# caojiezhang/CiaoSR

Measured on AMD Instinct MI355X. Metric: HR Mpix/s (RDN-CiaoSR x4, LocalImplicitSR forward_test), higher is better.
Workload: dtype f32; 1 GPU; C3: RDN-CiaoSR (c64b16) x4, LR 1356x2040 -> 5424x8160 (DIV2K-shaped 2K LR), tiled inference: 117 tiles of 192x192 (overlap 32), random-init weights, fp32; scale=4, tiles=117, parallelism=tile-shard x1

## Files before the change

ciaosr_amd/_lib.py:

```python
import ctypes as C
import os

_HERE = os.path.dirname(os.path.abspath(__file__))
LIB_PATH = os.environ.get('CIAOSR_HIP_LIB') or os.path.join(_HERE, 'csrc', 'libciaosr_hip.so')
MAX_LAYERS = 8

ACT_NONE, ACT_RELU, ACT_PRELU, ACT_GELU, ACT_SIN, ACT_COS = 0, 1, 2, 3, 4, 5


class CiaoSRHipError(RuntimeError):
    pass


class MlpT(C.Structure):
    _fields_ = [('n_layers', C.c_int), ('act', C.c_int), ('in_dim', C.c_int), ('width', C.c_int * MAX_LAYERS),
                ('weight', C.c_void_p * MAX_LAYERS), ('ld', C.c_int * MAX_LAYERS),
                ('bias', C.c_void_p * MAX_LAYERS), ('frag', C.c_void_p * MAX_LAYERS),
                ('frag16', C.c_void_p * MAX_LAYERS), ('frag16_lo', C.c_void_p * MAX_LAYERS)]


class HeadWeightsT(C.Structure):
    _fields_ = [('channels', C.c_int), ('nonlocal_channels', C.c_int), ('nonlocal_max_scale', C.c_int), ('local_size', C.c_int),
                ('no_unfold', C.c_int),
                ('softmax_scale', C.c_float), ('q', MlpT), ('k', MlpT), ('v', MlpT), ('k_out_wino', C.c_void_p), ('k_out_wino4', C.c_void_p),
                ('chain16', C.c_void_p), ('chain16_pairs', C.c_void_p)]


class HeadSceneT(C.Structure):
    _fields_ = [(n, C.c_int) for n in ('magic', 'H', 'W', 'C', 'Cn', 'D', 'Dv', 'J', 'q_plan', 'precision', 'route',
                                       'off_u', 'off_tk', 'off_tv', 'off_g', 'total')]


class CsAttnWeightsT(C.Structure):
    _fields_ = [('channels', C.c_int), ('scale', C.c_int),
                ('w_match1', C.c_void_p), ('b_match1', C.c_void_p), ('slope_match1', C.c_float),
                ('w_match2', C.c_void_p), ('b_match2', C.c_void_p), ('slope_match2', C.c_float),
                ('w_assembly', C.c_void_p), ('b_assembly', C.c_void_p), ('slope_assembly', C.c_float),
                ('w_down', C.c_void_p), ('b_down', C.c_void_p), ('w_down_masked', C.c_void_p),
                ('escape_nan', C.c_float), ('softmax_scale', C.c_float)]


class OptionsT(C.Structure):
    _fields_ = [('head_route', C.c_int), ('csa_composed_min', C.c_int), ('dense_min_tiles', C.c_int),
                ('scatter_small_max', C.c_int), ('kv_rows', C.c_int), ('decode_rows', C.c_int), ('bf16_single', C.c_int),
                ('dense_direct', C.c_int), ('csa_scores_gemm', C.c_int), ('csa_attn_tile128', C.c_int), ('query_grid_w', C.c_int), ('f16_pairs', C.c_int),
                ('csa_attn_v16', C.c_int), ('swin_h16', C.c_int), ('csa_block_mb', C.c_int)]


HEAD_STAGED, HEAD_NO_LOGIT_TABLE, HEAD_TABLE_GEMM, HEAD_WIDE_WG, HEAD_TABLE_WINO2, HEAD_NO_CHAIN, HEAD_NO_DECODE_CHAIN = 1, 2, 4, 8, 16, 32, 64


class ConvT(C.Structure):
    _fields_ = [('weight', C.c_void_p), ('bias', C.c_void_p), ('cin', C.c_int), ('cout', C.c_int), ('ksize', C.c_int),
                ('frag16', C.c_void_p), ('frag16_lo', C.c_void_p), ('frag', C.c_void_p), ('frag_wino', C.c_void_p),
                ('frag_wino4', C.c_void_p)]


class RdnWeightsT(C.Structure):
    _fields_ = [('mid_channels', C.c_int), ('growth', C.c_int), ('num_blocks', C.c_int), ('num_layers', C.c_int),
                ('sfe1', ConvT), ('sfe2', ConvT), ('gff0', ConvT), ('gff1', ConvT),
                ('dense', C.POINTER(ConvT)), ('lff', C.POINTER(ConvT)),
                ('scatter_weight', C.POINTER(C.c_void_p)), ('scatter_bias', C.c_void_p),
                ('scatter_frag', C.POINTER(C.c_void_p))]


class SwinBlockT(C.Structure):
    _fields_ = [(n, C.c_void_p) for n in ('ln1_w', 'ln1_b', 'qkv_w', 'qkv_b', 'bias', 'proj_w', 'proj_b', 'ln2_w', 'ln2_b',
                                           'fc1_w', 'fc1_b', 'fc2_w', 'fc2_b')] + [('shift', C.c_int), ('mask', C.c_void_p)] + \
               [(n, C.c_void_p) for n in ('qkv_w16', 'proj_w16', 'fc1_w16', 'fc2_w16')]


class SwinirWeightsT(C.Structure):
    _fields_ = [('embed_dim', C.c_int), ('num_heads', C.c_int), ('window_size', C.c_int), ('hidden', C.c_int),
                ('num_groups', C.c_int), ('depth', C.c_int), ('conv_first', ConvT), ('conv_after_body', ConvT),
                ('pe_norm_w', C.c_void_p), ('pe_norm_b', C.c_void_p), ('norm_w', C.c_void_p), ('norm_b', C.c_void_p),
                ('blocks', C.POINTER(SwinBlockT)), ('group_conv', C.POINTER(ConvT))]


class EdsrWeightsT(C.Structure):
    _fields_ = [('mid_channels', C.c_int), ('num_blocks', C.c_int), ('res_scale', C.c_float),
                ('conv_first', ConvT), ('conv_after_body', ConvT),
                ('conv1', C.POINTER(ConvT)), ('conv2', C.POINTER(ConvT))]
# ... 133 lines not shown
```

ciaosr_amd/csrc/common.h:

```cpp
#pragma once
#include <hip/hip_runtime.h>
#include <atomic>
#include <cstdint>
#include <cstdio>
#include <mutex>

#include "../../include/ciaosr_hip.h"

namespace ciaosr {

constexpr int kWave = 64;

static inline int ceil_div(long a, long b) { return (int)((a + b - 1) / b); }

static inline bool aligned16(const void* p) { return (reinterpret_cast<uintptr_t>(p) & 15u) == 0; }

struct ProfScope {
    int slot;
    hipStream_t stream;
    hipEvent_t ev0, ev1;
    ProfScope(const char* name, hipStream_t s);
    ~ProfScope();
};

constexpr int kMaxDevices = 32;
struct LdsAttrOnce {
    std::atomic<unsigned> granted[kMaxDevices];
    std::mutex raise;
};
template <typename K>
static inline bool allow_big_lds(LdsAttrOnce& once, K kernel, size_t bytes) {
    if (bytes <= 64 * 1024) return true;
    int dev = 0;
    if (hipGetDevice(&dev) != hipSuccess || dev < 0 || dev >= kMaxDevices) return false;
    if (once.granted[dev].load(std::memory_order_acquire) >= bytes) return true;
    std::lock_guard<std::mutex> lock(once.raise);
    if (once.granted[dev].load(std::memory_order_relaxed) >= bytes) return true;
    if (hipFuncSetAttribute(reinterpret_cast<const void*>(kernel), hipFuncAttributeMaxDynamicSharedMemorySize, (int)bytes) !=
        hipSuccess)
        return false;
    once.granted[dev].store((unsigned)bytes, std::memory_order_release);
    return true;
}

__device__ __forceinline__ void wave_lds_sync() {
    __builtin_amdgcn_fence(__ATOMIC_RELEASE, "wavefront");
    __builtin_amdgcn_wave_barrier();
    __builtin_amdgcn_fence(__ATOMIC_ACQUIRE, "wavefront");
}

int launch_status(const char* what);

static inline bool options_ok(const ciaosr_options_t* o) {
    if (!o) return true;
    return o->query_grid_w >= 0 && (o->csa_attn_tile128 == 0 || o->csa_attn_tile128 == 1) && (o->head_route & ~127) == 0 && (o->kv_rows == 0 || o->kv_rows == 32 || o->kv_rows == 64) &&
           (o->decode_rows == 0 || o->decode_rows == 32 || o->decode_rows == 64) && (o->bf16_single == 0 || o->bf16_single == 1) &&
           (o->dense_direct >= 0 && o->dense_direct <= 2) && (o->csa_scores_gemm == 0 || o->csa_scores_gemm == 1) &&
           o->f16_pairs >= 0 && o->f16_pairs <= 3 && (o->csa_attn_v16 == 0 || o->csa_attn_v16 == 1) && o->csa_block_mb >= 0 &&
           (o->swin_h16 == 0 || o->swin_h16 == 1);
}

}

#define CIAOSR_BIG_LDS(kernel, bytes)                                                              \
    do {                                                                                           \
        static ::ciaosr::LdsAttrOnce once_;                                                        \
        if (!::ciaosr::allow_big_lds(once_, kernel, bytes)) return CIAOSR_ERR_LAUNCH;              \
    } while (0)

#define CIAOSR_CHECK_ARG(cond)                                                         \
    do {                                                                               \
        if (!(cond)) {                                                                 \
            std::fprintf(stderr, "[ciaosr_hip] bad argument: %s (%s:%d)\n", #cond,     \
                         __FILE__, __LINE__);                                          \
            return CIAOSR_ERR_BAD_ARG;                                                 \
        }                                                                              \
    } while (0)
```

ciaosr_amd/csrc/head.hip:

```cpp
#include "ops.h"

namespace ciaosr {

struct HeadPlan {
    int H, W, C, Cn, D, Dv, J, HW;
    long Q;
    int wk0, wv0;
    int wmax;
    int qc;
    int qcf;
    size_t csa_bytes;
    size_t R() const { return (size_t)qc * J; }
};

constexpr int kLdG = 260;
constexpr int kQkChunk = 65536;

static int n_samples(int local_size) { return local_size == 1 ? 1 : (local_size == 2 ? 4 : 9); }

static HeadPlan head_plan(int H, int W, const ciaosr_head_weights_t* w, int Q, const ciaosr_options_t* opt) {
    HeadPlan p;
    p.H = H; p.W = W; p.C = w->channels; p.Cn = w->nonlocal_channels; p.Q = Q;
    p.D = (w->no_unfold ? 1 : 9) * p.C; p.Dv = p.D + p.Cn; p.J = n_samples(w->local_size); p.HW = H * W;
    p.wk0 = w->k.width[0];
// ... 75 lines not shown
    return {{round_up(a[0].off, 256), round_up(a[1].off, 256), round_up(a[2].off, 256)}};
}

static int mlp_act(const ciaosr_mlp_t& m) { return m.act == CIAOSR_ACT_SIN || m.act == CIAOSR_ACT_COS ? m.act : CIAOSR_ACT_RELU; }

static bool mlp_ok(const ciaosr_mlp_t& m) {
    if (m.n_layers < 1 || m.n_layers > CIAOSR_MAX_LAYERS) return false;
    for (int i = 0; i < m.n_layers; ++i)
        if (!m.weight[i] || !m.bias[i] || (m.ld[i] & 3) != 0 || m.width[i] <= 0) return false;
    return true;
}

static bool chain_fused_ok(const ciaosr_mlp_t& m, bool is_q, bool h16) {
    if (m.n_layers < 2 || mlp_act(m) != CIAOSR_ACT_RELU) return false;
    for (int i = 0; i + 1 < m.n_layers; ++i)
        if (m.width[i] != 256) return false;
    for (int i = is_q ? 0 : 1; i < m.n_layers - (is_q ? 1 : 0); ++i)
        if (!(h16 ? m.frag16[i] : (const void*)m.frag[i])) return false;
    return true;
}

enum HeadTables { kTablesH16, kTablesSmall, kTablesGemm };
enum HeadLogit { kLogitNone, kLogitGemm32, kLogitGemm16, kLogitWino2, kLogitWino4 };
enum HeadKernel { kHeadFused32, kHeadFused16, kHeadWide, kHeadChain };
struct HeadRoute {
    int refusal;
    bool fused;
    bool h16, lo;
    HeadTables tables;
    HeadLogit logit;
    HeadKernel kernel;
    int wide_mode;
    bool chain, decode_chain;
    HeadKernel kv(const HeadPlan& p, int nq) const { return chain && (size_t)nq * p.Dv * 2 < 0xFFFFFF00ull ? kHeadChain : kernel; }
    HeadKernel decode(const HeadPlan& p, int nq) const { return decode_chain && kv(p, nq) == kHeadChain ? kHeadChain : kernel; }
};

static HeadRoute head_route(const HeadPlan& p, Prec prec, const Mode& m, const ciaosr_options_t* opt, const ciaosr_head_weights_t* w) {
    const int bits = opt ? opt->head_route : 0;
    HeadRoute r = {CIAOSR_OK, false, prec != kF32, m.lo, kTablesGemm, kLogitNone, kHeadFused32, m.x3 ? 2 : (m.lo ? 1 : 0), false, false};
    r.fused = !(bits & CIAOSR_HEAD_STAGED) && w->local_size == 2 && chain_fused_ok(w->k, false, r.h16) && chain_fused_ok(w->v, false, r.h16) &&
              chain_fused_ok(w->q, true, r.h16) && (p.Dv & 7) == 0;
    if (r.h16 && !r.fused) r.refusal = CIAOSR_ERR_UNSUPPORTED;
    if (m.x3 && r.refusal == CIAOSR_OK) {
        bool all = true;
        for (int i = 1; i < w->k.n_layers; ++i) all = all && w->k.frag16_lo[i];
        for (int i = 1; i < w->v.n_layers; ++i) all = all && w->v.frag16_lo[i];
        for (int i = 0; i + 1 < w->q.n_layers; ++i) all = all && w->q.frag16_lo[i];
        if (!all) r.refusal = CIAOSR_ERR_BAD_ARG;
    }
    if (m.hoist16 && (p.D & 7) == 0 && (p.Dv & 7) == 0 && u16_fits(p)) r.tables = kTablesH16;
    else if (gemm_small_ok(p.HW, p.wk0, p.D, p.Dv, w->k.ld[0]) && gemm_small_ok(p.HW, p.wv0, p.Dv, p.Dv, w->v.ld[0]) && p.HW <= 4096)
        r.tables = kTablesSmall;
    const int last = w->k.n_layers - 1;
    if (r.fused && !(bits & CIAOSR_HEAD_NO_LOGIT_TABLE) && w->k.width[last] == p.D && w->k.width[last - 1] == 256 && p.Q * p.J > (long)p.HW * 9 &&
        (size_t)p.HW * 9 * kLdG * sizeof(float) < 0xFFFFFF00ull) {
        r.logit = m.table16 && (p.D & 7) == 0 ? kLogitGemm16 : kLogitGemm32;
        if (!m.table16 && w->k_out_wino && !(bits & CIAOSR_HEAD_TABLE_GEMM) && p.C == 64 && !w->no_unfold && p.HW >= 512 && qk_maps_fits(p))
            r.logit = w->k_out_wino4 && !(bits & CIAOSR_HEAD_TABLE_WINO2) ? kLogitWino4 : kLogitWino2;
    }
    if (!r.fused) return r;
    const bool wide = m.x3 || (prec == kF16 && (bits & CIAOSR_HEAD_WIDE_WG));
    r.kernel = wide ? kHeadWide : r.h16 ? kHeadFused16 : kHeadFused32;
    r.chain = r.kernel == kHeadFused16 && r.logit != kLogitNone && (m.lo ? w->chain16_pairs : w->chain16) && !(bits & CIAOSR_HEAD_NO_CHAIN) &&
              h16_ops(prec).head_chain_ok(w);
    r.decode_chain = r.chain && !(bits & CIAOSR_HEAD_NO_DECODE_CHAIN) && h16_ops(prec).head_decode_chain_ok(w);
    return r;
}

static int mlp_layers_f32(const ciaosr_mlp_t& m, int i0, int i1, const float* cur, int ld_cur, int k_cur, float* pp0, float* pp1, float* last_out,
                          int ld_last, long rows, hipStream_t s, const char* tag_first, const char* tag_hidden, const char* tag_out,
                          const float** end = nullptr) {
    float* pp[2] = {pp0, pp1};
    for (int i = i0; i < i1; ++i) {
        const bool last = i == m.n_layers - 1;
        float* dst = last ? last_out : pp[(i - i0) & 1];
        const int ldd = last ? ld_last : m.width[i];
        const int rc = gemm_f32(cur, ld_cur, m.weight[i], m.ld[i], false, dst, ldd, m.bias[i], (int)rows, m.width[i], k_cur, 1.f,
                                last ? CIAOSR_ACT_NONE : mlp_act(m), 0.f, s, last ? tag_out : i == i0 ? tag_first : tag_hidden);
        if (rc != CIAOSR_OK) return rc;
        cur = dst; ld_cur = ldd; k_cur = m.width[i];
    }
    if (end) *end = cur;
    return CIAOSR_OK;
}

template <class P>
static void fill_hidden(P& c, const ciaosr_mlp_t& m, const HeadRoute& r) {
    c.n_hidden = m.n_layers - 2;
    for (int i = 0; i < c.n_hidden; ++i) {
        c.frag_hidden[i] = r.h16 ? m.frag16[i + 1] : (const void*)m.frag[i + 1];
        c.frag_hidden_lo[i] = (r.h16 && r.lo) ? m.frag16_lo[i + 1] : nullptr;
        c.bias_hidden[i] = m.bias[i + 1];
    }
}
static void fill_chain(FusedChain& c, const ciaosr_mlp_t& m, const float* table, int fan, const HeadRoute& r) {
// ... 51 lines not shown
        const long total = (long)HW * 9;
        const float *w5 = w->k.weight[last], *b5 = w->k.bias[last];
        if (r.logit == kLogitWino4 || r.logit == kLogitWino2) {
            HEAD_RUN(ciaosr::qk_maps(feat, C, C, H, W, qk_maps(), s));
            HEAD_RUN(r.logit == kLogitWino4 ? wino4_table_f32(qk_maps(), H, W, w->k_out_wino4, 4, G, kLdG, s)
                                            : wino_table_f32(qk_maps(), H, W, w->k_out_wino, 4, G, kLdG, s));
            return qk_rows(U, Dv, D, H, W, 0, (int)total, b5, nullptr, G, kLdG, 3, s);
        }
        const bool t16 = r.logit == kLogitGemm16;
        if (t16) HEAD_RUN(transpose_cast_h16(w5, w->k.ld[last], D, 256, W5T, prec == kF16, s));
        for (long r0 = 0; r0 < total; r0 += kQkChunk) {
            const int nr = (int)((total - r0) < kQkChunk ? (total - r0) : kQkChunk);
            HEAD_RUN(qk_rows(U, Dv, D, H, W, r0, nr, b5, QK, G, kLdG, t16 ? (int)prec : 0, s));
            HEAD_RUN(t16 ? h16_ops(prec).gemm_nt(qk16(), D, W5T, D, G + (size_t)r0 * kLdG, kLdG, false, nr, 256, D, 1.f, s, kLogitTableTag16[prec], 0)
                         : gemm_f32(QK, D, w5, w->k.ld[last], true, G + (size_t)r0 * kLdG, kLdG, nullptr, nr, 256, D, 1.f, CIAOSR_ACT_NONE, 0.f, s,
                                    "head_logit_table"));
        }
        return CIAOSR_OK;
    }

    const void* chain_blob() const { return r.lo ? w->chain16_pairs : w->chain16; }
    int kv(long q0, int nq) const {
        FusedKVP kp;
        kp.coord = coord; kp.cell = cell; kp.q0 = q0; kp.nq = nq; kp.chunk = chunk; kp.H = H; kp.W = W;
        kp.U = U; kp.ldu = Dv; kp.D = D; kp.Dv = Dv;
        kp.u_bytes = (unsigned)((size_t)HW * Dv * sizeof(float));
        fill_chain(kp.k, w->k, Tk, D, r);
        fill_chain(kp.v, w->v, Tv, Dv, r);
        kp.softmax_scale = w->softmax_scale;
        kp.Z = Z; kp.ldz = Dv;
        kp.rows_per_wg = opt ? opt->kv_rows : 0;
        kp.G = r.logit != kLogitNone ? G : nullptr; kp.ldg = kLdG; kp.g_bytes = (unsigned)((size_t)HW * 9 * kLdG * sizeof(float));
        kp.gate = nullptr;
        if (r.kv(*this, nq) == kHeadChain) {
            if (hipMemsetAsync(chain_flag, 0, sizeof(int), s) != hipSuccess) return CIAOSR_ERR_LAUNCH;
            HEAD_RUN(h16_ops(prec).head_kv_chain(kp, w, chain_blob(), r.lo ? 1 : 0, opt ? opt->query_grid_w : 0, chain_flag, s));
            kp.gate = chain_flag;
        }
        if (r.kernel == kHeadWide) return h16_ops(prec).head_kv_fused_wide(kp, r.wide_mode, s);
        return r.kernel == kHeadFused16 ? h16_ops(prec).head_kv_fused(kp, s) : head_kv_fused(kp, s);
    }
    int decode(long q0, int nq) const {
        const ciaosr_mlp_t& mq = w->q;
        const int last = mq.n_layers - 1;
        FusedQP qp;
        qp.Z = Z; qp.ldz = Dv; qp.Dv = Dv;
        qp.frag_in = r.h16 ? mq.frag16[0] : (const void*)mq.frag[0]; qp.bias_in = mq.bias[0];
        qp.frag_in_lo = (r.h16 && r.lo) ? mq.frag16_lo[0] : nullptr;
        qp.nj_in = r.h16 ? (Dv + 15) / 16 : (Dv + 7) / 8;
        fill_hidden(qp, mq, r);
        qp.w_last = mq.weight[last]; qp.ld_last = mq.ld[last]; qp.b_last = mq.bias[last];
        qp.rows_per_wg = opt ? opt->decode_rows : 0;
        qp.x_lr = x_lr; qp.coord = coord; qp.q0 = q0; qp.nq = nq; qp.H = H; qp.W = W; qp.rgb = rgb;
        if (r.decode(*this, nq) == kHeadChain) {
            const H16Ops& h = h16_ops(prec);
            return h.head_decode_chain(qp, w, reinterpret_cast<const unsigned char*>(chain_blob()) + h.head_kv_chain_bytes(w, r.lo ? 1 : 0), r.lo ? 1 : 0, s);
        }
        if (r.kernel == kHeadWide) return h16_ops(prec).head_decode_fused_wide(qp, r.wide_mode, s);
        return r.kernel == kHeadFused16 ? h16_ops(prec).head_decode_fused(qp, s) : head_decode_fused(qp, s);
    }
    int staged_chunk(long q0, int nq) const {
        const long rows = (long)nq * J;
        HeadRowsP hp;
        hp.coord = coord; hp.cell = cell; hp.q0 = q0; hp.nq = nq; hp.chunk = chunk; hp.H = H; hp.W = W;
        hp.local_size = w->local_size; hp.J = J;
        hp.Tk = Tk; hp.Tv = Tv;
// ... 95 lines not shown
    CIAOSR_CHECK_ARG((size_t)p.HW * p.Dv * sizeof(float) < 0xFFFFFF00ull);
    Arena ar(workspace, workspace_bytes);
    const HeadCall c = {head_carve(p, nullptr, [&](Owner, size_t floats) { return ar.take<float>(floats); }), head_route(p, prec, resolve_mode(prec, opt), opt, w),
                        prec, feat_hwc, w, csattn, x_lr_nchw, coord, cell, chunk, rgb, opt, (hipStream_t)stream_};
    if (!ar.ok) return CIAOSR_ERR_WORKSPACE;
    HEAD_RUN(head_route_refusal(c.r));
    HEAD_RUN(c.per_image(n_scales));
    return c.per_query(Q);
}

extern "C" int ciaosr_head_forward_f32(const float* feat_hwc, int H, int W, const ciaosr_head_weights_t* w, const ciaosr_csattn_weights_t* csattn,
                                       const float* x_lr_nchw, const float* coord, const float* cell, int Q, int chunk, float* rgb, const ciaosr_options_t* opt,
                                       void* workspace, size_t workspace_bytes, void* stream) {
    return head_forward(feat_hwc, H, W, w, csattn, x_lr_nchw, coord, cell, Q, chunk, rgb, opt, workspace, workspace_bytes, stream, kF32);
}

extern "C" int ciaosr_head_forward_bf16(const float* feat_hwc, int H, int W, const ciaosr_head_weights_t* w, const ciaosr_csattn_weights_t* csattn,
                                        const float* x_lr_nchw, const float* coord, const float* cell, int Q, int chunk, float* rgb, const ciaosr_options_t* opt,
                                        void* workspace, size_t workspace_bytes, void* stream) {
    return head_forward(feat_hwc, H, W, w, csattn, x_lr_nchw, coord, cell, Q, chunk, rgb, opt, workspace, workspace_bytes, stream, kBF16);
}

extern "C" int ciaosr_head_forward_f16(const float* feat_hwc, int H, int W, const ciaosr_head_weights_t* w, const ciaosr_csattn_weights_t* csattn,
                                       const float* x_lr_nchw, const float* coord, const float* cell, int Q, int chunk, float* rgb, const ciaosr_options_t* opt,
                                       void* workspace, size_t workspace_bytes, void* stream) {
    return head_forward(feat_hwc, H, W, w, csattn, x_lr_nchw, coord, cell, Q, chunk, rgb, opt, workspace, workspace_bytes, stream, kF16);
}

constexpr int kSceneMagic = 0x43530001;

static int route_code(const HeadRoute& r) {
    if (r.refusal != CIAOSR_OK) return r.refusal;
    return (r.fused ? 1 : 0) | (int)r.tables << 1 | (int)r.logit << 3 | (int)r.kernel << 6 | (r.chain ? 1 : 0) << 8 | (r.decode_chain ? 1 : 0) << 9 |
           (r.h16 ? 1 : 0) << 10 | (r.lo ? 1 : 0) << 11 | r.wide_mode << 12;
}
static SceneLayout scene_layout(const HeadRoute& r) { return {r.logit != kLogitNone, r.tables == kTablesH16}; }

static int scene_route(int H, int W, const ciaosr_head_weights_t* w, int q_plan, Prec prec, const ciaosr_options_t* opt, HeadPlan* p, HeadRoute* r) {
    CIAOSR_CHECK_ARG(q_plan >= 1);
    HEAD_RUN(head_check_weights(H, W, w, opt));
    *p = head_plan(H, W, w, q_plan, opt);
    HEAD_RUN(head_check_dims(*p, w));
    CIAOSR_CHECK_ARG((size_t)p->HW * p->Dv * sizeof(float) < 0xFFFFFF00ull);
    *r = head_route(*p, prec, resolve_mode(prec, opt), opt, w);
    return head_route_refusal(*r);
}

extern "C" int ciaosr_head_route_code(int H, int W, const ciaosr_head_weights_t* w, int Q, int precision, const ciaosr_options_t* opt) {
    CIAOSR_CHECK_ARG(precision >= kF32 && precision <= kF16);
    HeadPlan p; HeadRoute r;
    HEAD_RUN(scene_route(H, W, w, Q, (Prec)precision, opt, &p, &r));
    return route_code(r);
}

static size_t scene_bytes_max(int H, int W, const ciaosr_head_weights_t* w, int q_plan, const ciaosr_options_t* opt, Owner o) {
    size_t n = 0;
    for (int prec = kF32; prec <= kF16; ++prec) {
        HeadPlan p; HeadRoute r;
        if (scene_route(H, W, w, q_plan, (Prec)prec, opt, &p, &r) != CIAOSR_OK) continue;
        const size_t m = head_split_bytes(p, scene_layout(r)).n[o];
        n = m > n ? m : n;
    }
    return n;
}
extern "C" size_t ciaosr_head_scene_bytes(int H, int W, const ciaosr_head_weights_t* w, int q_plan, const ciaosr_options_t* opt) {
    return scene_bytes_max(H, W, w, q_plan, opt, kScene);
}
// ... 201 lines not shown
```

ciaosr_amd/csrc/head_fused.hip:

```cpp

#include "h16_util.h"
#include "index_math.h"
#include "ops.h"

namespace ciaosr {

typedef float f32x16 __attribute__((ext_vector_type(16)));

constexpr int FH = 256;
constexpr int FLD = FH + 4;
constexpr int FNJ = FH / 8;

typedef int i32x4 __attribute__((ext_vector_type(4)));
constexpr unsigned kOobF = 0xFFFFFFF0u;

#ifdef CIAOSR_PROBE
__device__ unsigned long long g_hprobe[4096 * 16];
#define HPROBE(slot) do { if (threadIdx.x == 0 && blockIdx.x < 4096) g_hprobe[blockIdx.x * 16 + (slot)] = __builtin_readcyclecounter(); } while (0)
#else
#define HPROBE(slot) do { } while (0)
#endif

__device__ __forceinline__ float4 bload4(__amdgpu_buffer_rsrc_t rsrc, unsigned byte_off) {
    const i32x4 v = __builtin_amdgcn_raw_buffer_load_b128(rsrc, (int)byte_off, 0, 0);
// ... 150 lines not shown
__device__ __forceinline__ void hidden_layer(float* X, const void* __restrict__ frag, const float* __restrict__ bias,
                                             int w, int lane) {
    const int li = lane & 31, lh = lane >> 5;
    f32x16 acc[MT][2];
    bias_acc<MT>(acc, bias, w, lh);
    mma_pass_u<MT, 2, FNJ>(X + li * FLD + 4 * lh, frag_rsrc(frag), (unsigned)lane * 16u, (unsigned)(2 * w) * (FNJ * 1024u), FNJ * 1024u, acc);
    __syncthreads();
    store_relu_tile<MT>(X, acc, w, li, lh);
    __syncthreads();
}


template <int MT>
__device__ __forceinline__ void build_rows(float* X, const FusedChain& c, const int* s_kpix, const float* s_t4, int t) {
    const int n4 = t & 63;
    float4 tw[4];
#pragma unroll
    for (int e = 0; e < 4; ++e) tw[e] = *reinterpret_cast<const float4*>(c.tail + (size_t)(4 * n4 + e) * c.ld_tail);
    typedef float f32x2 __attribute__((ext_vector_type(2)));
    const f32x2 wy01 = {tw[0].x, tw[1].x}, wy23 = {tw[2].x, tw[3].x}, wx01 = {tw[0].y, tw[1].y}, wx23 = {tw[2].y, tw[3].y};
    const f32x2 vy01 = {tw[0].z, tw[1].z}, vy23 = {tw[2].z, tw[3].z}, vx01 = {tw[0].w, tw[1].w}, vx23 = {tw[2].w, tw[3].w};
    for (int r = t >> 6; r < 32 * MT; r += 4) {
        const float4 tv = reinterpret_cast<const float4*>(c.table + (size_t)s_kpix[r] * FH)[n4];
        const float4 t4 = *reinterpret_cast<const float4*>(s_t4 + 4 * r);
        const f32x2 ry = {t4.x, t4.x}, rx = {t4.y, t4.y}, sy = {t4.z, t4.z}, sx = {t4.w, t4.w};
        f32x2 a = __builtin_elementwise_fma(wy01, ry, f32x2{tv.x, tv.y}), b = __builtin_elementwise_fma(wy23, ry, f32x2{tv.z, tv.w});
        a = __builtin_elementwise_fma(wx01, rx, a); b = __builtin_elementwise_fma(wx23, rx, b);
        a = __builtin_elementwise_fma(vy01, sy, a); b = __builtin_elementwise_fma(vy23, sy, b);
        a = __builtin_elementwise_fma(vx01, sx, a); b = __builtin_elementwise_fma(vx23, sx, b);
        *reinterpret_cast<float4*>(X + r * FLD + 4 * n4) = make_float4(fmaxf(a.x, 0.f), fmaxf(a.y, 0.f), fmaxf(b.x, 0.f), fmaxf(b.y, 0.f));
    }
}


template <int MT>
__global__ __launch_bounds__(256, 2) void head_kv_fused_kernel(FusedKVP p) {
    constexpr int BM = 32 * MT;
    extern __shared__ __attribute__((aligned(16))) float smem[];
    float* X = smem;
    float* s_t4 = X + BM * FLD;
    float* s_part = s_t4 + BM * 4;
    float* s_attn = s_part + 4 * BM;
    int* s_kpix = reinterpret_cast<int*>(s_attn + BM);
    int* s_qpix = s_kpix + BM;
    int* s_goff = s_qpix + BM / 4;

    const int t = threadIdx.x, lane = t & 63, w = __builtin_amdgcn_readfirstlane(t >> 6);
    const int li = lane & 31, lh = lane >> 5;
    const int qbase = blockIdx.x * (BM / 4);
    HPROBE(0);

    int bad = 0;
    if (t < BM) {
        const int ql = qbase + (t >> 2), j = t & 3;
        int kpix = 0, goff = -1;
        float t4[4] = {0.f, 0.f, 0.f, 0.f};
        if (ql < p.nq) {
            const long q = p.q0 + ql;
            const float cy = p.coord[2 * q], cx = p.coord[2 * q + 1];
            const long c0 = p.chunk > 0 ? (q / p.chunk) * p.chunk : 0;
            const KeySample s = key_sample(cy, cx, p.cell[2 * c0], p.cell[2 * c0 + 1], p.H, p.W, j, 2);
            kpix = s.ky * p.W + s.kx;
            t4[0] = s.rel_y; t4[1] = s.rel_x;
            t4[2] = mul_rn(p.cell[2 * q], (float)p.H);
            t4[3] = mul_rn(p.cell[2 * q + 1], (float)p.W);
            const int iy = nearest_index(cy, p.H), ix = nearest_index(cx, p.W);
            const bool qin = iy >= 0 && iy < p.H && ix >= 0 && ix < p.W;
            if (j == 0) s_qpix[t >> 2] = qin ? iy * p.W + ix : -1;
            if (qin) {
                const int oy = s.ky - iy, ox = s.kx - ix;
                if (oy >= -1 && oy <= 1 && ox >= -1 && ox <= 1) goff = (iy * p.W + ix) * 9 + (oy + 1) * 3 + (ox + 1);
                else bad = 1;
            }
        } else if (j == 0) {
            s_qpix[t >> 2] = -1;
        }
        s_kpix[t] = kpix;
        s_goff[t] = goff;
#pragma unroll
        for (int e = 0; e < 4; ++e) s_t4[4 * t + e] = t4[e];
    }
    const bool table = p.G != nullptr && !__syncthreads_or(bad);
    if (p.G == nullptr) __syncthreads();

    HPROBE(1);
    build_rows<MT>(X, p.k, s_kpix, s_t4, t);
    __syncthreads();
    HPROBE(2);
    for (int l = 0; l < p.k.n_hidden; ++l) {
        hidden_layer<MT>(X, p.k.frag_hidden[l], p.k.bias_hidden[l], w, lane);
        if (l < 3) HPROBE(10 + l);
    }
    HPROBE(3);

    if (table) {
        const bool rv = (t >> 2) < BM;
        const int row = rv ? (t >> 2) : 0, part = t & 3;
        const int go = rv ? s_goff[row] : -1;
        const __amdgpu_buffer_rsrc_t rs_g = __builtin_amdgcn_make_buffer_rsrc(const_cast<float*>(p.G), 0, p.g_bytes, 0x00020000);
        const unsigned gbase = go >= 0 ? (unsigned)go * (unsigned)p.ldg * 4u : kOobF;
        float4 gv[16];
#pragma unroll
        for (int i = 0; i < 16; ++i) gv[i] = bload4(rs_g, gbase == kOobF ? kOobF : gbase + (unsigned)(16 * i + 4 * part) * 4u);
        const float cterm = (go >= 0 && part == 0) ? p.G[(size_t)go * p.ldg + 256] : 0.f;
        float a = 0.f;
#pragma unroll
        for (int i = 0; i < 16; ++i) {
            const float4 x = *reinterpret_cast<const float4*>(X + row * FLD + 16 * i + 4 * part);
            a += x.x * gv[i].x + x.y * gv[i].y + x.z * gv[i].z + x.w * gv[i].w;
        }
        a += cterm;
        a += quad_xor1(a);
        a += quad_xor2(a);
        if (part == 0 && rv) {
            s_part[row] = a;
            s_part[BM + row] = 0.f;
            s_part[2 * BM + row] = 0.f;
            s_part[3 * BM + row] = 0.f;
        }
    } else
    {
        float part[MT];
#pragma unroll
        for (int mi = 0; mi < MT; ++mi) part[mi] = 0.f;
        const int n_units = (p.k.n_out + 31) >> 5;
        const __amdgpu_buffer_rsrc_t rs_u = __builtin_amdgcn_make_buffer_rsrc(const_cast<float*>(p.U), 0, p.u_bytes, 0x00020000);
        const __amdgpu_buffer_rsrc_t rs_bk =
            __builtin_amdgcn_make_buffer_rsrc(const_cast<float*>(p.k.bias_out), 0, (unsigned)p.k.n_out * 4u, 0x00020000);
        unsigned koff[MT], qoff[MT];
#pragma unroll
        for (int mi = 0; mi < MT; ++mi) {
            const int m = 32 * mi + li;
            koff[mi] = (unsigned)s_kpix[m] * (unsigned)p.ldu * 4u;
            const int qp = s_qpix[m >> 2];
            qoff[mi] = qp >= 0 ? (unsigned)qp * (unsigned)p.ldu * 4u : kOobF;
        }
        for (int u = w; u < n_units; u += 4) {
            f32x16 acc[MT][1];
            zero_acc<MT, 1>(acc);
            mma_pass_u<MT, 1, FNJ>(X + li * FLD + 4 * lh, frag_rsrc(p.k.frag_out), (unsigned)lane * 16u, (unsigned)u * (FNJ * 1024u), 0u, acc);
            float4 bv[4], kv[MT][4], qv[MT][4];
#pragma unroll
            for (int g = 0; g < 4; ++g) {
                const int d0 = 32 * u + 8 * g + 4 * lh;
                const unsigned doff = d0 < p.k.n_out ? (unsigned)d0 * 4u : kOobF;
                bv[g] = bload4(rs_bk, doff);
#pragma unroll
                for (int mi = 0; mi < MT; ++mi) {
                    kv[mi][g] = bload4(rs_u, doff == kOobF ? kOobF : koff[mi] + doff);
                    qv[mi][g] = bload4(rs_u, (doff == kOobF || qoff[mi] == kOobF) ? kOobF : qoff[mi] + doff);
                }
            }
#pragma unroll
            for (int g = 0; g < 4; ++g)
#pragma unroll
                for (int mi = 0; mi < MT; ++mi)
                    part[mi] += qv[mi][g].x * (kv[mi][g].x * (acc[mi][0][4 * g] + bv[g].x)) +
                                qv[mi][g].y * (kv[mi][g].y * (acc[mi][0][4 * g + 1] + bv[g].y)) +
                                qv[mi][g].z * (kv[mi][g].z * (acc[mi][0][4 * g + 2] + bv[g].z)) +
                                qv[mi][g].w * (kv[mi][g].w * (acc[mi][0][4 * g + 3] + bv[g].w));
        }
#pragma unroll
        for (int mi = 0; mi < MT; ++mi) {
            part[mi] += __shfl_xor(part[mi], 32, 64);
            if (lh == 0) s_part[w * BM + 32 * mi + li] = part[mi];
        }
    }
    __syncthreads();
    if (t < BM / 4) {
        float lg[4], m = -INFINITY;
#pragma unroll
        for (int j = 0; j < 4; ++j) {
            const int row = 4 * t + j;
            lg[j] = (s_part[row] + s_part[BM + row] + s_part[2 * BM + row] + s_part[3 * BM + row]) / p.softmax_scale;
            m = fmaxf(m, lg[j]);
        }
        float den = 0.f;
#pragma unroll
        for (int j = 0; j < 4; ++j) { lg[j] = expf(lg[j] - m); den += lg[j]; }
#pragma unroll
        for (int j = 0; j < 4; ++j) s_attn[4 * t + j] = lg[j] / den;
    }

    HPROBE(4);
    build_rows<MT>(X, p.v, s_kpix, s_t4, t);
    __syncthreads();
    HPROBE(5);
    for (int l = 0; l < p.v.n_hidden; ++l) {
        hidden_layer<MT>(X, p.v.frag_hidden[l], p.v.bias_hidden[l], w, lane);
        if (l < 3) HPROBE(13 + l);
    }
    HPROBE(6);
    {
        const int n_units = (p.v.n_out + 31) >> 5;
        const __amdgpu_buffer_rsrc_t rs_u = __builtin_amdgcn_make_buffer_rsrc(const_cast<float*>(p.U), 0, p.u_bytes, 0x00020000);
        const __amdgpu_buffer_rsrc_t rs_bv =
            __builtin_amdgcn_make_buffer_rsrc(const_cast<float*>(p.v.bias_out), 0, (unsigned)p.v.n_out * 4u, 0x00020000);
        const __amdgpu_buffer_rsrc_t rs_z =
            __builtin_amdgcn_make_buffer_rsrc(p.Z, 0, (unsigned)((size_t)p.nq * p.ldz * 4), 0x00020000);
        unsigned voff[MT], zoff[MT];
        float av[MT];
        const int jsel = li & 3;
#pragma unroll
        for (int mi = 0; mi < MT; ++mi) {
            const int m = 32 * mi + li;
            voff[mi] = (unsigned)s_kpix[m] * (unsigned)p.ldu * 4u;
            av[mi] = s_attn[m];
            const int ql = qbase + (m >> 2);
            zoff[mi] = ql < p.nq ? (unsigned)ql * (unsigned)p.ldz * 4u : kOobF;
        }
        for (int u = w; u < n_units; u += 4) {
            float4 bv[4], vv[MT][4];
#pragma unroll
            for (int g = 0; g < 4; ++g) {
                const int d0 = 32 * u + 8 * g + 4 * lh;
                const unsigned doff = d0 < p.v.n_out ? (unsigned)d0 * 4u : kOobF;
                bv[g] = bload4(rs_bv, doff);
#pragma unroll
// ... 113 lines not shown
            const float y0f = floorf(fy), x0f = floorf(fx);
            const int y0 = (int)y0f, x0 = (int)x0f;
            const float wy1 = fy - y0f, wy0 = (y0f + 1.f) - fy;
            const float wx1 = fx - x0f, wx0 = (x0f + 1.f) - fx;
            const float* img = p.x_lr + (size_t)part * p.H * p.W;
            const bool y1ok = y0 + 1 < p.H, x1ok = x0 + 1 < p.W;
            float r = img[(size_t)y0 * p.W + x0] * (wx0 * wy0);
            if (x1ok) r += img[(size_t)y0 * p.W + x0 + 1] * (wx1 * wy0);
            if (y1ok) r += img[(size_t)(y0 + 1) * p.W + x0] * (wx0 * wy1);
            if (y1ok && x1ok) r += img[(size_t)(y0 + 1) * p.W + x0 + 1] * (wx1 * wy1);
            v += r;
        }
        p.rgb[q * 3 + part] = v;
    }
}

size_t fragment_floats(int N, int K) { return (size_t)((N + 31) / 32) * ((K + 7) / 8) * 64 * 4; }

int pack_fragments(const float* W, int ld, int N, int K, float* P, hipStream_t s) {
    const int n_tiles = (N + 31) / 32, nj = (K + 7) / 8;
    const long total = (long)n_tiles * nj * 64;
    int grid = (int)((total + 255) / 256);
    ProfScope prof("pack_fragments", s);
    hipLaunchKernelGGL(pack_fragments_kernel, dim3(grid > 4096 ? 4096 : grid), dim3(256), 0, s, W, ld, N, K, P, n_tiles, nj);
    return launch_status("pack_fragments");
}

template <int MT>
constexpr size_t fused_kv_lds() {
    return (size_t)(32 * MT * FLD + 32 * MT * 4 + 4 * 32 * MT + 32 * MT) * sizeof(float) + (32 * MT + 8 * MT + 32 * MT) * sizeof(int);
}

int head_kv_fused(const FusedKVP& p, hipStream_t s) {
    CIAOSR_BIG_LDS(head_kv_fused_kernel<1>, fused_kv_lds<1>());
    CIAOSR_BIG_LDS(head_kv_fused_kernel<2>, fused_kv_lds<2>());
    const int rows = p.rows_per_wg == 64 || (p.rows_per_wg != 32 && ceil_div(p.nq, 16) >= 2048) ? 64 : 32;
    ProfScope prof("head_kv_fused", s);
    if (rows == 64)
        hipLaunchKernelGGL(head_kv_fused_kernel<2>, dim3(ceil_div(p.nq, 16)), dim3(256), fused_kv_lds<2>(), s, p);
    else
        hipLaunchKernelGGL(head_kv_fused_kernel<1>, dim3(ceil_div(p.nq, 8)), dim3(256), fused_kv_lds<1>(), s, p);
    return launch_status("head_kv_fused");
}

int head_decode_fused(const FusedQP& p, hipStream_t s) {
    CIAOSR_BIG_LDS(head_decode_fused_kernel<2>, (size_t)64 * FLD * sizeof(float));
    CIAOSR_BIG_LDS(head_decode_fused_kernel<1>, (size_t)32 * FLD * sizeof(float));
    const int rows = p.rows_per_wg == 64 ? 64 : 32;
    ProfScope prof("head_decode_fused", s);
    if (rows == 64)
        hipLaunchKernelGGL(head_decode_fused_kernel<2>, dim3(ceil_div(p.nq, 64)), dim3(256), (size_t)64 * FLD * sizeof(float), s, p);
    else
        hipLaunchKernelGGL(head_decode_fused_kernel<1>, dim3(ceil_div(p.nq, 32)), dim3(256), (size_t)32 * FLD * sizeof(float), s, p);
    return launch_status("head_decode_fused");
}

}

using namespace ciaosr;

extern "C" size_t ciaosr_fragment_floats(int N, int K) { return fragment_floats(N, K); }

extern "C" int ciaosr_pack_fragments_f32(const float* W, int ld, int N, int K, float* out, void* stream) {
    CIAOSR_CHECK_ARG(W && out && N > 0 && K > 0 && ld >= K);
    return pack_fragments(W, ld, N, K, out, (hipStream_t)stream);
}

#ifdef CIAOSR_PROBE
extern "C" int ciaosr_debug_probe_read(unsigned long long* host, int n_words) {
    return hipMemcpyFromSymbol(host, HIP_SYMBOL(ciaosr::g_hprobe), (size_t)n_words * 8) == hipSuccess ? 0 : -1;
}
#endif
```

ciaosr_amd/csrc/ops.h:

```cpp
#pragma once
#include "common.h"

namespace ciaosr {

constexpr int MAXJ = 9;

struct HeadRowsP {
    const float* coord;
    const float* cell;
    long q0;
    int nq, chunk, H, W, local_size, J;
    const float* Tk;
    const float* Tv;
    const float* tailK;
    const float* tailV;
    int ld_tail_k, ld_tail_v;
    int wk0, wv0, relu_k, relu_v;
    float* Hk;
    float* Hv;
    int* q_idx;
    int* k_idx;
};

struct LocalAttnP {
// ... 81 lines not shown
int local_attention(const LocalAttnP& p, hipStream_t s);
int decode_residual(const DecodeP& p, hipStream_t s);

struct FusedChain {
    const float* table;
    const float* tail;
    int ld_tail;
    const void* frag_hidden[CIAOSR_MAX_LAYERS];
    const void* frag_hidden_lo[CIAOSR_MAX_LAYERS];
    const float* bias_hidden[CIAOSR_MAX_LAYERS];
    int n_hidden;
    const void* frag_out;
    const void* frag_out_lo;
    const float* bias_out;
    int n_out;
};
struct FusedKVP {
    const float* coord;
    const float* cell;
    long q0;
    int nq, chunk, H, W;
    const float* U;
    int ldu, D, Dv;
    unsigned u_bytes;
    FusedChain k, v;
    float softmax_scale;
    float* Z;
    int ldz;
    const float* G;
    int ldg;
    unsigned g_bytes;
    int rows_per_wg;
    const int* gate;
};
struct FusedQP {
    const float* Z; int ldz, Dv;
    const void* frag_in;
    const void* frag_in_lo;
    const float* bias_in;
    int nj_in;
    const void* frag_hidden[CIAOSR_MAX_LAYERS];
    const void* frag_hidden_lo[CIAOSR_MAX_LAYERS];
    const float* bias_hidden[CIAOSR_MAX_LAYERS];
    int n_hidden;
    const float* w_last; int ld_last;
    const float* b_last;
    const float* x_lr;
    const float* coord;
    long q0;
    int nq, H, W;
    float* rgb;
    int rows_per_wg;
};
int head_kv_fused(const FusedKVP& p, hipStream_t s);
int head_decode_fused(const FusedQP& p, hipStream_t s);

#define CIAOSR_H16_DECLS                                                                                                              \
    int gemm_h16_nt(const unsigned short* A, int lda, const unsigned short* B, int ldb, void* C, int ldc, bool c_bf16, int M, int N,  \
                    int K, float alpha, hipStream_t s, const char* tag, int plan_rows );                    \
    int cast_rows_h16(const float* src, int ld_src, unsigned short* dst, int ld_dst, long rows, int cols, hipStream_t s);             \
    int linear_h16(const unsigned short* A, int lda, const unsigned short* W16, int ldw, const float* bias, bool relu, void* C, int ldc,      \
                   bool c_16bit, int M, int N, int K, hipStream_t s, const char* tag);                                                      \
    int softmax_rows_h16(const float* S, long rows, int L, int ld, unsigned short* P, int ldp, hipStream_t s);                        \
    int head_kv_fused_h16(const FusedKVP& p, hipStream_t s);                                                                          \
    int head_decode_fused_h16(const FusedQP& p, hipStream_t s);                                                                       \
    bool head_chain_ok(const ciaosr_head_weights_t* w);                                                                               \
// ... 111 lines not shown
```

include/ciaosr_hip.h:

```cpp
#ifndef CIAOSR_HIP_H
#define CIAOSR_HIP_H

#include <stddef.h>

#ifdef __cplusplus
extern "C" {
#endif

#define CIAOSR_OK 0
#define CIAOSR_ERR_BAD_ARG (-1)
#define CIAOSR_ERR_LAUNCH (-2)
#define CIAOSR_ERR_UNSUPPORTED (-3)
#define CIAOSR_ERR_WORKSPACE (-4)

#define CIAOSR_ACT_NONE 0
#define CIAOSR_ACT_RELU 1
#define CIAOSR_ACT_PRELU 2
#define CIAOSR_ACT_GELU 3
#define CIAOSR_ACT_SIN 4
#define CIAOSR_ACT_COS 5

#define CIAOSR_MAX_LAYERS 8

int ciaosr_version(void);
const char* ciaosr_error_string(int code);
size_t ciaosr_sizeof(const char* type_name );

int ciaosr_prof_enable(int on);
int ciaosr_prof_filter(const char* kernel );
int ciaosr_prof_reset(void);
int ciaosr_prof_collect(void);
int ciaosr_prof_get(const char* kernel, double* total_ms , long* launches );
int ciaosr_prof_names(char* buf , int buflen);

#define CIAOSR_HEAD_STAGED 1
#define CIAOSR_HEAD_TABLE_GEMM 4
#define CIAOSR_HEAD_NO_LOGIT_TABLE 2
#define CIAOSR_HEAD_WIDE_WG 8
#define CIAOSR_HEAD_TABLE_WINO2 16
#define CIAOSR_HEAD_NO_CHAIN 32
#define CIAOSR_HEAD_NO_DECODE_CHAIN 64
typedef struct ciaosr_options {
    int head_route;
    int csa_composed_min;
    int dense_min_tiles;
    int scatter_small_max;
    int kv_rows;
    int decode_rows;
    int bf16_single;
    int dense_direct;
    int csa_scores_gemm;
    int csa_attn_tile128;
    int query_grid_w;
    int f16_pairs;
    int csa_attn_v16;
    int swin_h16;
    int csa_block_mb;
} ciaosr_options_t;

int ciaosr_nchw_to_hwc_f32(const float* src, float* dst, int C, int H, int W, int ld_dst, void* stream);
int ciaosr_hwc_to_nchw_f32(const float* src, int ld_src, float* dst, int C, int H, int W, void* stream);

int ciaosr_gemm_f32(const float* A, int lda, const float* B, int ldb, int b_is_kn, float* C, int ldc,
                    const float* bias, int M, int N, int K, float alpha, int act, float slope,
                    void* stream);

int ciaosr_patch_rows_f32(const float* src_hwc, int ld_src, int Hs, int Ws, int Cs, int ksize, int stride,
                          int pad, int OH, int OW, float* out, int ld_out, int l2_normalize,
                          float norm_floor, void* stream);

typedef struct ciaosr_csattn_weights {
    int channels;
    int scale;
// ... 272 lines not shown
```

Measured before the change: 11.97 Mpix/s.

## Prefetch K/V table rows and logit gathers ahead of MLP layers in fused head kernel

Splits the row-building gather in the fused fp32 head KV kernel into a request phase (buffer loads into registers) and a finish phase (FMA+ReLU into LDS). The V-table gathers and the logit-table G loads are issued early so they overlap the last K hidden layer and the score reduction instead of being serialised. The old serial path stays behind a new route bit and is forced when the table size would overflow 32-bit buffer offsets. The cost is many more live VGPRs (extra float4 arrays held across layers), which could lower occupancy or cause spills under the 256x2 launch bounds.

Result: no change. 12.09 Mpix/s (median of 6 runs) (+1.0%).

```diff
diff --git a/ciaosr_amd/_lib.py b/ciaosr_amd/_lib.py
--- a/ciaosr_amd/_lib.py
+++ b/ciaosr_amd/_lib.py
@@ -48,6 +48,7 @@
 
 
 HEAD_STAGED, HEAD_NO_LOGIT_TABLE, HEAD_TABLE_GEMM, HEAD_WIDE_WG, HEAD_TABLE_WINO2, HEAD_NO_CHAIN, HEAD_NO_DECODE_CHAIN = 1, 2, 4, 8, 16, 32, 64
+HEAD_SERIAL_GATHERS = 128
 
 
 class ConvT(C.Structure):
diff --git a/ciaosr_amd/csrc/common.h b/ciaosr_amd/csrc/common.h
--- a/ciaosr_amd/csrc/common.h
+++ b/ciaosr_amd/csrc/common.h
@@ -53,7 +53,7 @@
 
 static inline bool options_ok(const ciaosr_options_t* o) {
     if (!o) return true;
-    return o->query_grid_w >= 0 && (o->csa_attn_tile128 == 0 || o->csa_attn_tile128 == 1) && (o->head_route & ~127) == 0 && (o->kv_rows == 0 || o->kv_rows == 32 || o->kv_rows == 64) &&
+    return o->query_grid_w >= 0 && (o->csa_attn_tile128 == 0 || o->csa_attn_tile128 == 1) && (o->head_route & ~255) == 0 && (o->kv_rows == 0 || o->kv_rows == 32 || o->kv_rows == 64) &&
            (o->decode_rows == 0 || o->decode_rows == 32 || o->decode_rows == 64) && (o->bf16_single == 0 || o->bf16_single == 1) &&
            (o->dense_direct >= 0 && o->dense_direct <= 2) && (o->csa_scores_gemm == 0 || o->csa_scores_gemm == 1) &&
            o->f16_pairs >= 0 && o->f16_pairs <= 3 && (o->csa_attn_v16 == 0 || o->csa_attn_v16 == 1) && o->csa_block_mb >= 0 &&
diff --git a/ciaosr_amd/csrc/head.hip b/ciaosr_amd/csrc/head.hip
--- a/ciaosr_amd/csrc/head.hip
+++ b/ciaosr_amd/csrc/head.hip
@@ -131,13 +131,14 @@
     HeadKernel kernel;
     int wide_mode;
     bool chain, decode_chain;
+    bool serial_gathers;
     HeadKernel kv(const HeadPlan& p, int nq) const { return chain && (size_t)nq * p.Dv * 2 < 0xFFFFFF00ull ? kHeadChain : kernel; }
     HeadKernel decode(const HeadPlan& p, int nq) const { return decode_chain && kv(p, nq) == kHeadChain ? kHeadChain : kernel; }
 };
 
 static HeadRoute head_route(const HeadPlan& p, Prec prec, const Mode& m, const ciaosr_options_t* opt, const ciaosr_head_weights_t* w) {
     const int bits = opt ? opt->head_route : 0;
-    HeadRoute r = {CIAOSR_OK, false, prec != kF32, m.lo, kTablesGemm, kLogitNone, kHeadFused32, m.x3 ? 2 : (m.lo ? 1 : 0), false, false};
+    HeadRoute r = {CIAOSR_OK, false, prec != kF32, m.lo, kTablesGemm, kLogitNone, kHeadFused32, m.x3 ? 2 : (m.lo ? 1 : 0), false, false, false};
     r.fused = !(bits & CIAOSR_HEAD_STAGED) && w->local_size == 2 && chain_fused_ok(w->k, false, r.h16) && chain_fused_ok(w->v, false, r.h16) &&
               chain_fused_ok(w->q, true, r.h16) && (p.Dv & 7) == 0;
     if (r.h16 && !r.fused) r.refusal = CIAOSR_ERR_UNSUPPORTED;
@@ -161,6 +162,7 @@
     if (!r.fused) return r;
     const bool wide = m.x3 || (prec == kF16 && (bits & CIAOSR_HEAD_WIDE_WG));
     r.kernel = wide ? kHeadWide : r.h16 ? kHeadFused16 : kHeadFused32;
+    r.serial_gathers = r.kernel == kHeadFused32 && ((bits & CIAOSR_HEAD_SERIAL_GATHERS) || (size_t)p.HW * 256 * sizeof(float) >= 0xFFFFFF00ull);
     r.chain = r.kernel == kHeadFused16 && r.logit != kLogitNone && (m.lo ? w->chain16_pairs : w->chain16) && !(bits & CIAOSR_HEAD_NO_CHAIN) &&
               h16_ops(prec).head_chain_ok(w);
     r.decode_chain = r.chain && !(bits & CIAOSR_HEAD_NO_DECODE_CHAIN) && h16_ops(prec).head_decode_chain_ok(w);
@@ -278,6 +280,7 @@
         kp.rows_per_wg = opt ? opt->kv_rows : 0;
         kp.G = r.logit != kLogitNone ? G : nullptr; kp.ldg = kLdG; kp.g_bytes = (unsigned)((size_t)HW * 9 * kLdG * sizeof(float));
         kp.gate = nullptr;
+        kp.serial_gathers = r.serial_gathers ? 1 : 0;
         if (r.kv(*this, nq) == kHeadChain) {
             if (hipMemsetAsync(chain_flag, 0, sizeof(int), s) != hipSuccess) return CIAOSR_ERR_LAUNCH;
             HEAD_RUN(h16_ops(prec).head_kv_chain(kp, w, chain_blob(), r.lo ? 1 : 0, opt ? opt->query_grid_w : 0, chain_flag, s));
@@ -439,7 +442,7 @@
 static int route_code(const HeadRoute& r) {
     if (r.refusal != CIAOSR_OK) return r.refusal;
     return (r.fused ? 1 : 0) | (int)r.tables << 1 | (int)r.logit << 3 | (int)r.kernel << 6 | (r.chain ? 1 : 0) << 8 | (r.decode_chain ? 1 : 0) << 9 |
-           (r.h16 ? 1 : 0) << 10 | (r.lo ? 1 : 0) << 11 | r.wide_mode << 12;
+           (r.h16 ? 1 : 0) << 10 | (r.lo ? 1 : 0) << 11 | r.wide_mode << 12 | (r.serial_gathers ? 1 : 0) << 14;
 }
 static SceneLayout scene_layout(const HeadRoute& r) { return {r.logit != kLogitNone, r.tables == kTablesH16}; }
 
diff --git a/ciaosr_amd/csrc/head_fused.hip b/ciaosr_amd/csrc/head_fused.hip
--- a/ciaosr_amd/csrc/head_fused.hip
+++ b/ciaosr_amd/csrc/head_fused.hip
@@ -206,8 +206,51 @@
     }
 }
 
-
-template <int MT>
+template <int MT>
+__device__ __forceinline__ void request_rows(float4 (&tv)[8 * MT], float4 (&tw)[4], const FusedChain& c, unsigned table_bytes, const int* s_kpix, int t) {
+    const __amdgpu_buffer_rsrc_t rs_t = __builtin_amdgcn_make_buffer_rsrc(const_cast<float*>(c.table), 0, table_bytes, 0x00020000);
+    const int n4 = t & 63;
+    const __amdgpu_buffer_rsrc_t rs_w =
+        __builtin_amdgcn_make_buffer_rsrc(const_cast<float*>(c.tail), 0, (unsigned)((FH - 1) * c.ld_tail + 4) * 4u, 0x00020000);
+    int kp[8 * MT];
+#pragma unroll
+    for (int s = 0; s < 8 * MT; ++s) kp[s] = s_kpix[(t >> 6) + 4 * s];
+    __builtin_amdgcn_sched_barrier(0);
+#pragma unroll
+    for (int e = 0; e < 4; ++e) tw[e] = bload4(rs_w, (unsigned)((4 * n4 + e) * c.ld_tail) * 4u);
+#pragma unroll
+    for (int s = 0; s < 8 * MT; ++s) tv[s] = bload4(rs_t, (unsigned)kp[s] * (unsigned)(FH * 4) + (unsigned)n4 * 16u);
+    __builtin_amdgcn_sched_barrier(0);
+}
+
+template <int MT>
+__device__ __forceinline__ void finish_rows(float* X, const float4 (&tvs)[8 * MT], const float4 (&tw_)[4], const float* s_t4, int t) {
+    const int n4 = t & 63;
+    float4 tw[4];
+#pragma unroll
+    for (int e = 0; e < 4; ++e) {
+        tw[e] = tw_[e];
+        asm("" : "+v"(tw[e].x)); asm("" : "+v"(tw[e].y)); asm("" : "+v"(tw[e].z)); asm("" : "+v"(tw[e].w));
+    }
+    typedef float f32x2 __attribute__((ext_vector_type(2)));
+    const f32x2 wy01 = {tw[0].x, tw[1].x}, wy23 = {tw[2].x, tw[3].x}, wx01 = {tw[0].y, tw[1].y}, wx23 = {tw[2].y, tw[3].y};
+    const f32x2 vy01 = {tw[0].z, tw[1].z}, vy23 = {tw[2].z, tw[3].z}, vx01 = {tw[0].w, tw[1].w}, vx23 = {tw[2].w, tw[3].w};
+#pragma unroll
+    for (int s = 0; s < 8 * MT; ++s) {
+        const int r = (t >> 6) + 4 * s;
+        const float4 tv = tvs[s];
+        const float4 t4 = *reinterpret_cast<const float4*>(s_t4 + 4 * r);
+        const f32x2 ry = {t4.x, t4.x}, rx = {t4.y, t4.y}, sy = {t4.z, t4.z}, sx = {t4.w, t4.w};
+        f32x2 a = __builtin_elementwise_fma(wy01, ry, f32x2{tv.x, tv.y}), b = __builtin_elementwise_fma(wy23, ry, f32x2{tv.z, tv.w});
+        a = __builtin_elementwise_fma(wx01, rx, a); b = __builtin_elementwise_fma(wx23, rx, b);
+        a = __builtin_elementwise_fma(vy01, sy, a); b = __builtin_elementwise_fma(vy23, sy, b);
+        a = __builtin_elementwise_fma(vx01, sx, a); b = __builtin_elementwise_fma(vx23, sx, b);
+        *reinterpret_cast<float4*>(X + r * FLD + 4 * n4) = make_float4(fmaxf(a.x, 0.f), fmaxf(a.y, 0.f), fmaxf(b.x, 0.f), fmaxf(b.y, 0.f));
+    }
+}
+
+
+template <int MT, bool SERIAL>
 __global__ __launch_bounds__(256, 2) void head_kv_fused_kernel(FusedKVP p) {
     constexpr int BM = 32 * MT;
     extern __shared__ __attribute__((aligned(16))) float smem[];
@@ -258,25 +301,55 @@
     if (p.G == nullptr) __syncthreads();
 
     HPROBE(1);
-    build_rows<MT>(X, p.k, s_kpix, s_t4, t);
+    constexpr bool G_AHEAD = !SERIAL && MT == 2;
+    const unsigned table_bytes = (unsigned)(p.H * p.W) * (unsigned)(FH * 4);
+    if constexpr (SERIAL) {
+        build_rows<MT>(X, p.k, s_kpix, s_t4, t);
+    } else {
+        float4 tv[8 * MT], tw[4];
+        request_rows<MT>(tv, tw, p.k, table_bytes, s_kpix, t);
+        finish_rows<MT>(X, tv, tw, s_t4, t);
+    }
     __syncthreads();
     HPROBE(2);
-    for (int l = 0; l < p.k.n_hidden; ++l) {
+    const bool rv = (t >> 2) < BM;
+    const int row = rv ? (t >> 2) : 0, part = t & 3;
+    float4 gv[16];
+    float cterm = 0.f;
+#define CIAOSR_REQUEST_G()                                                                                                             \
+    {                                                                                                                                  \
+        const int go = rv ? s_goff[row] : -1;                                                                                          \
+        const __amdgpu_buffer_rsrc_t rs_g = __builtin_amdgcn_make_buffer_rsrc(const_cast<float*>(p.G), 0, p.g_bytes, 0x00020000);      \
+        const unsigned gbase = go >= 0 ? (unsigned)go * (unsigned)p.ldg * 4u : kOobF;                                                  \
+        _Pragma("unroll") for (int i = 0; i < 16; ++i)                                                                                 \
+            gv[i] = bload4(rs_g, gbase == kOobF ? kOobF : gbase + (unsigned)(16 * i + 4 * part) * 4u);                                  \
+        if constexpr (SERIAL) cterm = (go >= 0 && part == 0) ? p.G[(size_t)go * p.ldg + 256] : 0.f;                                    \
+        else cterm = __int_as_float(__builtin_amdgcn_raw_buffer_load_b32(rs_g, (int)((gbase == kOobF || part != 0) ? kOobF : gbase + 256u * 4u), 0, 0)); \
+    }
+    const int nk = p.k.n_hidden;
+    for (int l = 0; l + 1 < nk; ++l) {
         hidden_layer<MT>(X, p.k.frag_hidden[l], p.k.bias_hidden[l], w, lane);
         if (l < 3) HPROBE(10 + l);
     }
+    if constexpr (G_AHEAD) {
+        if (p.G != nullptr) CIAOSR_REQUEST_G()
+        __builtin_amdgcn_sched_barrier(0);
+    }
+    if (nk > 0) {
+        hidden_layer<MT>(X, p.k.frag_hidden[nk - 1], p.k.bias_hidden[nk - 1], w, lane);
+        if (nk - 1 < 3) HPROBE(10 + nk - 1);
+    }
     HPROBE(3);
+    constexpr bool V_AHEAD = !SERIAL && MT == 2;
+    float4 tvv[8 * MT], twv[4];
 
     if (table) {
-        const bool rv = (t >> 2) < BM;
-        const int row = rv ? (t >> 2) : 0, part = t & 3;
-        const int go = rv ? s_goff[row] : -1;
-        const __amdgpu_buffer_rsrc_t rs_g = __builtin_amdgcn_make_buffer_rsrc(const_cast<float*>(p.G), 0, p.g_bytes, 0x00020000);
-        const unsigned gbase = go >= 0 ? (unsigned)go * (unsigned)p.ldg * 4u : kOobF;
-        float4 gv[16];
-#pragma unroll
-        for (int i = 0; i < 16; ++i) gv[i] = bload4(rs_g, gbase == kOobF ? kOobF : gbase + (unsigned)(16 * i + 4 * part) * 4u);
-        const float cterm = (go >= 0 && part == 0) ? p.G[(size_t)go * p.ldg + 256] : 0.f;
+        if constexpr (V_AHEAD) {
+            request_rows<MT>(tvv, twv, p.v, table_bytes, s_kpix, t);
+            __builtin_amdgcn_sched_barrier(0);
+        }
+        if constexpr (!G_AHEAD) CIAOSR_REQUEST_G()
+#undef CIAOSR_REQUEST_G
         float a = 0.f;
 #pragma unroll
         for (int i = 0; i < 16; ++i) {
@@ -339,7 +412,9 @@
             part[mi] += __shfl_xor(part[mi], 32, 64);
             if (lh == 0) s_part[w * BM + 32 * mi + li] = part[mi];
         }
-    }
+        if constexpr (V_AHEAD) request_rows<MT>(tvv, twv, p.v, table_bytes, s_kpix, t);
+    }
+    if constexpr (!SERIAL && !V_AHEAD) request_rows<MT>(tvv, twv, p.v, table_bytes, s_kpix, t);
     __syncthreads();
     if (t < BM / 4) {
         float lg[4], m = -INFINITY;
@@ -357,7 +432,8 @@
     }
 
     HPROBE(4);
-    build_rows<MT>(X, p.v, s_kpix, s_t4, t);
+    if constexpr (SERIAL) build_rows<MT>(X, p.v, s_kpix, s_t4, t);
+    else finish_rows<MT>(X, tvv, twv, s_t4, t);
     __syncthreads();
     HPROBE(5);
     for (int l = 0; l < p.v.n_hidden; ++l) {
@@ -537,14 +613,20 @@
 }
 
 int head_kv_fused(const FusedKVP& p, hipStream_t s) {
-    CIAOSR_BIG_LDS(head_kv_fused_kernel<1>, fused_kv_lds<1>());
-    CIAOSR_BIG_LDS(head_kv_fused_kernel<2>, fused_kv_lds<2>());
+    CIAOSR_BIG_LDS((head_kv_fused_kernel<1, false>), fused_kv_lds<1>());
+    CIAOSR_BIG_LDS((head_kv_fused_kernel<2, false>), fused_kv_lds<2>());
+    CIAOSR_BIG_LDS((head_kv_fused_kernel<1, true>), fused_kv_lds<1>());
+    CIAOSR_BIG_LDS((head_kv_fused_kernel<2, true>), fused_kv_lds<2>());
     const int rows = p.rows_per_wg == 64 || (p.rows_per_wg != 32 && ceil_div(p.nq, 16) >= 2048) ? 64 : 32;
     ProfScope prof("head_kv_fused", s);
-    if (rows == 64)
-        hipLaunchKernelGGL(head_kv_fused_kernel<2>, dim3(ceil_div(p.nq, 16)), dim3(256), fused_kv_lds<2>(), s, p);
+    if (rows == 64 && p.serial_gathers)
+        hipLaunchKernelGGL((head_kv_fused_kernel<2, true>), dim3(ceil_div(p.nq, 16)), dim3(256), fused_kv_lds<2>(), s, p);
+    else if (rows == 64)
+        hipLaunchKernelGGL((head_kv_fused_kernel<2, false>), dim3(ceil_div(p.nq, 16)), dim3(256), fused_kv_lds<2>(), s, p);
+    else if (p.serial_gathers)
+        hipLaunchKernelGGL((head_kv_fused_kernel<1, true>), dim3(ceil_div(p.nq, 8)), dim3(256), fused_kv_lds<1>(), s, p);
     else
-        hipLaunchKernelGGL(head_kv_fused_kernel<1>, dim3(ceil_div(p.nq, 8)), dim3(256), fused_kv_lds<1>(), s, p);
+        hipLaunchKernelGGL((head_kv_fused_kernel<1, false>), dim3(ceil_div(p.nq, 8)), dim3(256), fused_kv_lds<1>(), s, p);
     return launch_status("head_kv_fused");
 }
 
diff --git a/ciaosr_amd/csrc/ops.h b/ciaosr_amd/csrc/ops.h
--- a/ciaosr_amd/csrc/ops.h
+++ b/ciaosr_amd/csrc/ops.h
@@ -137,6 +137,7 @@
     unsigned g_bytes;
     int rows_per_wg;
     const int* gate;
+    int serial_gathers;
 };
 struct FusedQP {
     const float* Z; int ldz, Dv;
diff --git a/include/ciaosr_hip.h b/include/ciaosr_hip.h
--- a/include/ciaosr_hip.h
+++ b/include/ciaosr_hip.h
@@ -39,6 +39,7 @@
 #define CIAOSR_HEAD_WIDE_WG 8
 #define CIAOSR_HEAD_TABLE_WINO2 16
 #define CIAOSR_HEAD_NO_CHAIN 32
+#define CIAOSR_HEAD_SERIAL_GATHERS 128
 #define CIAOSR_HEAD_NO_DECODE_CHAIN 64
 typedef struct ciaosr_options {
     int head_route;
```
